# langtech-bsc/quantool

Measured on AMD Instinct MI355X. Metric: quantized weights/sec (GPTQ int4, Llama-3-8B, 512 calib samples), higher is better.
Workload: dtype f32

## Files before the change

quantool_amd/csrc/build.py:

```python
from __future__ import annotations

import hashlib
import os
import shutil
import subprocess
import sys
from concurrent.futures import ThreadPoolExecutor
from pathlib import Path

CSRC = Path(__file__).resolve().parent
PKG = CSRC.parent
LIB_DIR = PKG / "lib"
OBJ_DIR = CSRC / "_obj"
LIB_PATH = LIB_DIR / "libquantool_hip.so"

HIPCC_FLAGS = [
    "--offload-arch=gfx950",
    "-O3",
    "-fPIC",
    "-std=c++17",
    "-ffp-contract=off",
    "-fhip-fp32-correctly-rounded-divide-sqrt",
    "-fno-fast-math",
    "-Wall",
# ... 55 lines not shown
        if m:
            kv = m.group(1).strip()
            if kv.startswith("Function Name:"):
                cur = {"name": kv.split(":", 1)[1].strip()}
                kernels.append(cur)
            elif cur is not None and ":" in kv:
                k, v = kv.rsplit(":", 1)
                cur[k.strip()] = v.strip()
            while i + 1 < len(lines) and re.match(r"^\s+\d* ?\|", lines[i + 1]):
                i += 1
        elif not re.match(r"^\d+ (warning|remark)s? generated", line.strip()) and "remarks generated" not in line:
            rest.append(line)
        i += 1
    rows = []
    for k in kernels:
        rows.append(f"{k['name']}\tvgpr {k.get('VGPRs', '?')}\tagpr {k.get('AGPRs', '?')}\tscratch "
                    f"{k.get('ScratchSize [bytes/lane]', '?')}\tvgpr_spill {k.get('VGPRs Spill', '?')}\tlds "
                    f"{k.get('LDS Size [bytes/block]', '?')}\twaves_per_simd {k.get('Occupancy [waves/SIMD]', '?')}")
    (OBJ_DIR / (src.stem + ".resources.txt")).write_text("\n".join(rows) + ("\n" if rows else ""))
    bad = [k["name"] for k in kernels
           if k.get("ScratchSize [bytes/lane]", "0") not in ("0", "?") and not any(ok in k["name"] for ok in SCRATCH_OK)]
    if bad:
        raise RuntimeError(f"{src.name}: kernel(s) with a private segment (scratch): {bad} -- see "
                           f"{OBJ_DIR / (src.stem + '.resources.txt')}; a by-value argument struct that is modified and "
                           "indexed at run time, or a register array indexed at run time, is the usual cause")
    return "\n".join(rest) + ("\n" if rest else "")


def audit_m0(src: Path) -> None:
    stamp = OBJ_DIR / (src.stem + ".m0audit")
    want = _stamp(src)
    if stamp.exists() and stamp.read_text() == want:
        return
    asm = OBJ_DIR / (src.stem + ".device.s")
    cmd = [_hipcc(), *[f for f in HIPCC_FLAGS if f != "-fPIC"], "--cuda-device-only", "-S", str(src), "-o", str(asm)]
    res = subprocess.run(cmd, capture_output=True, text=True)
    if res.returncode != 0:
        raise RuntimeError(f"hipcc -S failed for {src.name}:\n{res.stderr}")
    inside = False
    for n, line in enumerate(asm.read_text().splitlines(), 1):
        if ";;#ASMSTART" in line:
            inside = True
        elif ";;#ASMEND" in line:
            inside = False
        elif not inside and "m0" in line.split(";")[0].replace("_m0", ""):
            raise RuntimeError(f"{src.name}: compiler-generated use of M0 at {asm.name}:{n}: {line.strip()!r} -- "
                               "the LDS-DMA helpers must save/restore M0 again")
    audit_spills(src.name, asm.read_text())
    asm.unlink()
    stamp.write_text(want)


NO_SPILL_KERNELS = ("xtx_kernel", "xtx16_kernel", "gemm3_kernel", "sgemm_ring_kernel", "quantize_tokens_kernel",
                    "gemm_i8_kernel")


def audit_spills(src_name: str, asm_text: str) -> None:
    name = None
    for line in asm_text.splitlines():
        t = line.strip()
        if t.startswith(".name:"):
            name = t.split(":", 1)[1].strip()
        elif name and t.startswith((".vgpr_spill_count:", ".private_segment_fixed_size:")):
            if int(t.split(":", 1)[1]) != 0 and any(k in name for k in NO_SPILL_KERNELS):
                raise RuntimeError(f"{src_name}: {name} spills ({t}) -- its schedule assumes every value stays in registers")


def build(verbose: bool = False) -> Path:
    OBJ_DIR.mkdir(exist_ok=True)
    LIB_DIR.mkdir(exist_ok=True)
    srcs = sources()
    with ThreadPoolExecutor(max_workers=min(8, len(srcs))) as ex:
        objs = list(ex.map(_compile, srcs))
    for name in ("xtx.hip", "gemm3_tn.hip", "sgemm_tn.hip", "qlinear.hip"):
        audit_m0(CSRC / name)
    newest = max(o.stat().st_mtime for o in objs)
    if not LIB_PATH.exists() or LIB_PATH.stat().st_mtime < newest:
        cmd = [_hipcc(), "--offload-arch=gfx950", "-shared", "-fPIC", "-o", str(LIB_PATH), *map(str, objs)]
        res = subprocess.run(cmd, capture_output=True, text=True)
        if res.returncode != 0:
            raise RuntimeError(f"link failed:\n{res.stdout}\n{res.stderr}")
    if verbose:
        print(f"built {LIB_PATH}")
    return LIB_PATH


if __name__ == "__main__":
    build(verbose=True)
```

quantool_amd/csrc/cholesky.hip:

```cpp
#include <stdlib.h>
#include <string.h>

#include <map>
#include <tuple>
#include <vector>

#include "common.h"
#include "gemm3_tn.h"
#include "sgemm_tn.h"

namespace {

constexpr int NB = 128;
constexpr int NBO_MAX = 1024;
static int chol_block_env(const char* name) {
    const char* e = getenv(name);
    if (!e) return 0;
    int x = atoi(e) / 128 * 128;
    return x < 128 ? 128 : (x > NBO_MAX ? NBO_MAX : x);
}
struct G3Step {
    int n_items = 0, n_red = 0;
    size_t item_off = 0, red_off = 0;
};
// ... 47 lines not shown
        for (const G3Red& r : red) pl->max_slabs = pl->max_slabs > r.first + r.count ? pl->max_slabs : r.first + r.count;
        pl->any = true;
        return st;
    };
    for (int J0 = 0; J0 < K; J0 += NBO) {
        const int J1 = (K - J0 < NBO) ? K : J0 + NBO;
        pl->fac.push_back(J0 == 0 ? G3Step() : add((J1 - J0 + 255) / 256, (K - J0 + 255) / 256, J0 / G3_CHUNK_ROWS, 0));
    }
    for (int I0 = 0; I0 < K; I0 += NBI) {
        const int I1 = (K - I0 < NBI) ? K : I0 + NBI;
        pl->inv.push_back(I0 == 0 ? G3Step() : add((I1 - I0 + 255) / 256, (I0 + 255) / 256, I0 / G3_CHUNK_ROWS, 1));
    }
    if (pl->any) {
        pl->blob_bytes = qt_align_up(bytes.size(), 256);
        if (hipHostMalloc((void**)&pl->blob, pl->blob_bytes, hipHostMallocDefault) != hipSuccess) {
            pl->any = false;
            pl->blob = nullptr;
        } else {
            memcpy(pl->blob, bytes.data(), bytes.size());
        }
    }
    if (!pl->any) {
        pl->blob_bytes = 0;
        pl->max_slabs = 0;
        for (G3Step& st : pl->fac) st = G3Step();
        for (G3Step& st : pl->inv) st = G3Step();
    }
    plans[key] = pl;
    return pl;
}
static size_t chol_g3_ws_bytes(const CholG3Plan* pl, int K) {
    if (!pl->any) return 0;
    return 2 * qt_align_up((size_t)3 * K * K * 2, 256) + (size_t)pl->max_slabs * 256 * 256 * 4 + pl->blob_bytes + 256;
}

static const CholG3Plan* chol_blocks(int K, int& NBO, int& NBI) {
    const int eo = chol_block_env("QT_CHOL_NBO"), ei = chol_block_env("QT_CHOL_NBI");
    NBO = eo ? eo : 512;
    NBI = ei ? ei : 512;
    const CholG3Plan* pl = chol_g3_plan(K, NBO, NBI);
    if (pl->any) return pl;
    NBO = eo ? eo : 256;
    NBI = ei ? ei : 256;
    return chol_g3_plan(K, NBO, NBI);
}

constexpr int LDP = NB + 1;

constexpr int LDT = NB + 4;
constexpr int RD_STRIDE = NB * NB + 4 * 32 * 32;

#define QT_SEL4(kb, v0, v1, v2, v3) ((kb) == 0 ? (v0) : (kb) == 1 ? (v1) : (kb) == 2 ? (v2) : (v3))

constexpr int LDA = NB + 4;

__device__ __forceinline__ float readlane_f(float v, int lane) {
    return __int_as_float(__builtin_amdgcn_readlane(__float_as_int(v), lane));
}

__device__ __forceinline__ void mma32_tn(const float* A, int lda, const float* B, int ldb, f32x16& acc,
                                         int l31, int h, bool negate_a) {
#pragma unroll
    for (int kk = 0; kk < 16; ++kk) {
        float a = A[(2 * kk + h) * lda + l31];
        const float b = B[(2 * kk + h) * ldb + l31];
        if (negate_a) a = -a;
        acc = __builtin_amdgcn_mfma_f32_32x32x2f32(a, b, acc, 0, 0, 0);
    }
}

constexpr int POTF2_THREADS = 512, POTF2_WAVES = POTF2_THREADS / 64;
__global__ __launch_bounds__(POTF2_THREADS) void potf2_kernel(const float* P, int64_t ldp, int n,
                                                    float* Rout, int64_t ldr,
                                                    float* __restrict__ Rd, int32_t* info, int col0, int prio,
                                                    int64_t bsP, int64_t bsRd) {
    qt_set_chain_prio(prio);
    if (blockIdx.x) {
        P += (size_t)blockIdx.x * bsP;
        Rout += (size_t)blockIdx.x * bsP;
        Rd += (size_t)blockIdx.x * bsRd;
        info += blockIdx.x;
    }
    extern __shared__ __attribute__((aligned(16))) float sm[];
    float* As = sm;
    float* Xs = sm + NB * LDA;
    const int tid = threadIdx.x, lane = tid & 63;
    const int wave = __builtin_amdgcn_readfirstlane(tid >> 6);
    const int l31 = lane & 31, h = lane >> 5;

    if ((ldp & 3) == 0 && (n & 3) == 0 && (((uintptr_t)P) & 15) == 0) {
        constexpr int NV = NB * NB / 4 / POTF2_THREADS;
        f32x4 v[NV];
#pragma unroll
        for (int r = 0; r < NV; ++r) {
            const int e4 = tid + POTF2_THREADS * r;
            const int i = e4 >> 5, j = (e4 & 31) * 4;
            const int ic = i < n ? i : n - 1, jc = j < n ? j : n - 4;
            v[r] = *(const f32x4*)(P + (size_t)ic * ldp + jc);
        }
#pragma unroll
        for (int r = 0; r < NV; ++r) {
            const int e4 = tid + POTF2_THREADS * r;
            const int i = e4 >> 5, j = (e4 & 31) * 4;
            f32x4 x;
#pragma unroll
            for (int q = 0; q < 4; ++q) x[q] = (i < n && j + q < n) ? v[r][q] : (i == j + q ? 1.0f : 0.0f);
            *(f32x4*)(As + i * LDA + j) = x;
        }
    } else {
        for (int e = tid; e < NB * NB; e += POTF2_THREADS) {
            const int i = e / NB, j = e % NB;
            const int lo = i < j ? i : j, hi = i < j ? j : i;
            float v = (i == j) ? 1.0f : 0.0f;
            if (hi < n) v = P[(size_t)lo * ldp + hi];
            As[i * LDA + j] = v;
        }
    }
    __syncthreads();

    int bad = 0;
#pragma unroll 1
    for (int kb = 0; kb < 4; ++kb) {
        float* Akk = As + (32 * kb) * LDA + 32 * kb;
        if (wave == 0) {
            f32x16 c1, c2;
#pragma unroll
            for (int r = 0; r < 16; ++r) {
                const int i = (r & 3) + 8 * (r >> 2) + 4 * h;
                c1[r] = Akk[i * LDA + l31];
                c2[r] = (i == l31) ? 1.0f : 0.0f;
            }
#pragma unroll
            for (int c = 0; c < 32; ++c) {
                const int rc = (c & 3) + 4 * (c >> 3);
                const int hc = (c >> 2) & 1;
                float piv = readlane_f(c1[rc], c + 32 * hc);
                const bool isbad = !(piv > 0.0f);
                bad = (isbad && bad == 0 && 32 * kb + c < n) ? 32 * kb + c + 1 : bad;
                piv = isbad ? 1.0f : piv;
                float rs = __builtin_amdgcn_rsqf(piv);
                rs = rs * fmaf(-0.5f * piv * rs, rs, 1.5f);
                const bool mine = h == hc;
                const float rr = c1[rc] * rs, zz = c2[rc] * rs;
                c1[rc] = mine ? rr : c1[rc];
                c2[rc] = mine ? zz : c2[rc];
                if (c < 31) {
                    const float a = (mine && l31 > c) ? -rr : 0.0f;
                    const float b1 = (mine && l31 >= c) ? rr : 0.0f, b2 = mine ? zz : 0.0f;
                    c1 = __builtin_amdgcn_mfma_f32_32x32x2f32(a, b1, c1, 0, 0, 0);
                    c2 = __builtin_amdgcn_mfma_f32_32x32x2f32(a, b2, c2, 0, 0, 0);
                }
            }
#pragma unroll
            for (int r = 0; r < 16; ++r) {
                const int i = (r & 3) + 8 * (r >> 2) + 4 * h;
                Akk[i * LDA + l31] = (i <= l31) ? c1[r] : 0.0f;
                Xs[(kb * 32 + l31) * 32 + i] = (i >= l31) ? c2[r] : 0.0f;
            }
        }
        __syncthreads();
        if (kb == 3) break;
        for (int a = kb + 1 + wave; a < 4; a += POTF2_WAVES) {
            f32x16 acc;
#pragma unroll
            for (int r = 0; r < 16; ++r) acc[r] = 0.0f;
            float* Bt = As + (32 * kb) * LDA + 32 * a;
            mma32_tn(Xs + kb * 1024, 32, Bt, LDA, acc, l31, h, false);
#pragma unroll
            for (int r = 0; r < 16; ++r) Bt[((r & 3) + 8 * (r >> 2) + 4 * h) * LDA + l31] = acc[r];
        }
        __syncthreads();
        {
            int t = 0;
            for (int a = kb + 1; a < 4; ++a)
                for (int a2 = a; a2 < 4; ++a2, ++t) {
                    if ((t % POTF2_WAVES) != wave) continue;
                    float* Ct = As + (32 * a) * LDA + 32 * a2;
                    f32x16 acc;
#pragma unroll
                    for (int r = 0; r < 16; ++r) acc[r] = Ct[((r & 3) + 8 * (r >> 2) + 4 * h) * LDA + l31];
                    mma32_tn(As + (32 * kb) * LDA + 32 * a, LDA, As + (32 * kb) * LDA + 32 * a2, LDA, acc, l31, h,
                             true);
#pragma unroll
                    for (int r = 0; r < 16; ++r) Ct[((r & 3) + 8 * (r >> 2) + 4 * h) * LDA + l31] = acc[r];
                }
        }
        __syncthreads();
    }
    if (bad != 0 && tid == 0) atomicCAS(info, 0, col0 + bad);
    const bool vec_out = (ldr & 3) == 0 && (n & 3) == 0 && (((uintptr_t)Rout) & 15) == 0;
    for (int e4 = tid; e4 < NB * NB / 4; e4 += POTF2_THREADS) {
        const int i = e4 >> 5, j = (e4 & 31) * 4;
        f32x4 v = *(const f32x4*)(As + i * LDA + j);
#pragma unroll
        for (int q = 0; q < 4; ++q) v[q] = (j + q >= i) ? v[q] : 0.0f;
        *(f32x4*)(Rd + i * NB + j) = v;
        if (i < n && j + 3 >= i && j < n) {
            if (vec_out) {
                *(f32x4*)(Rout + (size_t)i * ldr + j) = v;
            } else {
#pragma unroll
                for (int q = 0; q < 4; ++q)
                    if (j + q >= i && j + q < n) Rout[(size_t)i * ldr + j + q] = v[q];
            }
        }
    }
    for (int e4 = tid; e4 < 4 * 32 * 32 / 4; e4 += POTF2_THREADS) *(f32x4*)(Rd + NB * NB + 4 * e4) = *(const f32x4*)(Xs + 4 * e4);
}

__global__ __launch_bounds__(256) void trsm_rt_kernel(const float* __restrict__ Rd, int n,
                                                      const float* B, int64_t ldb,
                                                      float* Z, int64_t ldz, int ncols, int prio, int64_t bsRd,
                                                      int64_t bsB) {
    qt_set_chain_prio(prio);
    if (blockIdx.y) {
        Rd += (size_t)blockIdx.y * bsRd;
        B += (size_t)blockIdx.y * bsB;
        Z += (size_t)blockIdx.y * bsB;
    }
    extern __shared__ __attribute__((aligned(16))) float Rs[];
    const int tid = threadIdx.x, lane = tid & 63, wave = tid >> 6;
    const float* D32 = Rs + NB * NB;
    const int l31 = lane & 31, h = lane >> 5;
    const int col = blockIdx.x * 128 + wave * 32 + l31;
    const bool cok = col < ncols;
    const int colc = cok ? col : ncols - 1;

    f32x16 acc[4];
#pragma unroll
    for (int a = 0; a < 4; ++a)
#pragma unroll
        for (int r = 0; r < 16; ++r) {
            const int row = 32 * a + (r & 3) + 8 * (r >> 2) + 4 * h;
            acc[a][r] = (row < n) ? B[(size_t)row * ldb + colc] : 0.0f;
        }
    {
        constexpr int NV = RD_STRIDE / 4 / 256;
        static_assert(NV * 4 * 256 == RD_STRIDE, "whole float4s per thread");
        f32x4 v[NV];
#pragma unroll
        for (int r = 0; r < NV; ++r) v[r] = ((const f32x4*)Rd)[tid + 256 * r];
#pragma unroll
        for (int r = 0; r < NV; ++r) ((f32x4*)Rs)[tid + 256 * r] = v[r];
    }
    __syncthreads();

#pragma unroll
    for (int b = 0; b < 4; ++b) {
        f32x16 zb;
#pragma unroll
        for (int r = 0; r < 16; ++r) zb[r] = 0.0f;
#pragma unroll
        for (int r = 0; r < 16; ++r) {
            const int k = (r & 3) + 8 * (r >> 2) + 4 * h;
            const float av = D32[(b * 32 + k) * 32 + l31];
            zb = __builtin_amdgcn_mfma_f32_32x32x2f32(av, acc[b][r], zb, 0, 0, 0);
        }
        acc[b] = zb;
#pragma unroll
        for (int a = b + 1; a < 4; ++a) {
#pragma unroll
            for (int r = 0; r < 16; ++r) {
                const int k = (r & 3) + 8 * (r >> 2) + 4 * h;
                const float av = -Rs[(32 * b + k) * NB + 32 * a + l31];
                acc[a] = __builtin_amdgcn_mfma_f32_32x32x2f32(av, zb[r], acc[a], 0, 0, 0);
            }
        }
    }
    if (cok) {
#pragma unroll
        for (int a = 0; a < 4; ++a)
#pragma unroll
            for (int r = 0; r < 16; ++r) {
                const int row = 32 * a + (r & 3) + 8 * (r >> 2) + 4 * h;
                if (row < n) Z[(size_t)row * ldz + col] = acc[a][r];
            }
    }
}

__global__ __launch_bounds__(128) void trinv_batched_kernel(const float* __restrict__ Rd_all, int K,
                                                            float* __restrict__ Dinv_all,
                                                            float* __restrict__ Y, int64_t ldy, int64_t bsW, int64_t bsY) {
    if (blockIdx.y) {
        Rd_all += (size_t)blockIdx.y * bsW;
        Dinv_all += (size_t)blockIdx.y * bsW;
        Y += (size_t)blockIdx.y * bsY;
    }
    extern __shared__ __attribute__((aligned(16))) float sm[];
    float* Rt = sm;
    float* Xs = sm + NB * LDT;
    const int b = blockIdx.x;
    const int n = (K - b * NB < NB) ? K - b * NB : NB;
    const float* Rd = Rd_all + (size_t)b * RD_STRIDE;
    const int j = threadIdx.x;
    for (int e = j; e < NB * NB; e += NB) {
        const int i = e / NB, c = e % NB;
        Rt[c * LDT + i] = Rd[e];
    }
    __syncthreads();
    float x0[32], x1[32], x2[32], x3[32];
#pragma unroll
    for (int r = 0; r < 32; ++r) {
        x0[r] = (r == j) ? 1.0f : 0.0f;
        x1[r] = (32 + r == j) ? 1.0f : 0.0f;
        x2[r] = (64 + r == j) ? 1.0f : 0.0f;
        x3[r] = (96 + r == j) ? 1.0f : 0.0f;
    }
#pragma unroll 1
    for (int pb = 3; pb >= 0; --pb) {
#pragma unroll
        for (int pp = 31; pp >= 0; --pp) {
            const int p = 32 * pb + pp;
            const float* rp = Rt + p * LDT;
            const float xp = QT_SEL4(pb, x0[pp], x1[pp], x2[pp], x3[pp]) / rp[p];
            if (pb == 0) x0[pp] = xp;
            if (pb == 1) x1[pp] = xp;
            if (pb == 2) x2[pp] = xp;
            if (pb == 3) x3[pp] = xp;
#define QT_XUPD(arr, a, r_to)                                                 \
    _Pragma("unroll") for (int r4 = 0; r4 < (r_to); r4 += 4) {                 \
        const f32x4 v4 = *(const f32x4*)(rp + 32 * (a) + r4);                 \
        _Pragma("unroll") for (int e = 0; e < 4; ++e)                         \
            if (r4 + e < (r_to)) arr[r4 + e] = fmaf(-v4[e], xp, arr[r4 + e]); \
    }
            if (pb == 0) { QT_XUPD(x0, 0, pp) } else { QT_XUPD(x0, 0, 32) }
            if (pb == 1) { QT_XUPD(x1, 1, pp) } else if (pb > 1) { QT_XUPD(x1, 1, 32) }
            if (pb == 2) { QT_XUPD(x2, 2, pp) } else if (pb > 2) { QT_XUPD(x2, 2, 32) }
            if (pb == 3) { QT_XUPD(x3, 3, pp) }
#undef QT_XUPD
        }
// ... 179 lines not shown
    const size_t split_ws_bytes = (size_t)2048 * NB * NB * 4 + (size_t)NBO_MAX * K * 4;
    unsigned short *Rpl = nullptr, *Ypl = nullptr;
    float* g3_slabs = nullptr;
    char* g3_tab = nullptr;
    const int64_t plane_stride = (int64_t)K * K;
    if (g3->any) {
        char* q = (char*)qt_align_up((size_t)((char*)split_ws + split_ws_bytes), 256);
        Rpl = (unsigned short*)q;
        q += qt_align_up((size_t)3 * K * K * 2, 256);
        Ypl = (unsigned short*)q;
        q += qt_align_up((size_t)3 * K * K * 2, 256);
        g3_slabs = (float*)q;
        g3_tab = (char*)qt_align_up((size_t)(ws + (size_t)nprob * prob_bytes), 256);
        QT_HIP(hipMemcpyAsync(g3_tab, g3->blob, g3->blob_bytes, hipMemcpyHostToDevice, stream));
    }
    auto g3_row = [&](const G3Step& st, const unsigned short* Bplanes, int col_a0, int col_b0, int M, int N, float* C,
                      int64_t bsC, int mode) -> int {
        G3Args a;
        a.Apl = Rpl;
        a.Bpl = Bplanes;
        a.plane_stride = plane_stride;
        a.ld = K;
        a.rowA0 = a.rowB0 = 0;
        a.colA0 = col_a0;
        a.colB0 = col_b0;
        a.colmax = K;
        a.M = M;
        a.N = N;
        a.C = C;
        a.ldc = K;
        a.mode = mode;
        a.slabs = g3_slabs;
        a.items = (const G3Item*)(g3_tab + st.item_off);
        a.n_items = st.n_items;
        a.red = (const G3Red*)(g3_tab + st.red_off);
        a.n_red = st.n_red;
        a.batch = nprob;
        a.bsApl = a.bsBpl = sW * 2;
        a.bsC = bsC;
        a.bsSlabs = sW;
        return qt_gemm3_launch(a, stream);
    };
    auto sgemm = [&](SgemmArgs& g, int64_t bsA_, int64_t bsB_, int64_t bsC_) -> int {
        g.batch = nprob;
        g.bsA = bsA_;
        g.bsB = bsB_;
        g.bsCin = g.bsCout = bsC_;
        g.bs_split = sW;
        return qt_sgemm_tn(g, stream);
    };
    float* Y = U;
    const int64_t sY = sU;
    const size_t inv_lds = (size_t)(NB * LDT + NB * LDP) * sizeof(float);
    const size_t potf2_lds = (size_t)(NB * LDA + 4 * 32 * 32) * sizeof(float);
    static QtOncePerDevice lds_attr;
    QT_HIP(lds_attr.run([&] {
        hipError_t e = hipFuncSetAttribute((const void*)potf2_kernel, hipFuncAttributeMaxDynamicSharedMemorySize,
                                           (int)potf2_lds);
        if (e == hipSuccess)
            e = hipFuncSetAttribute((const void*)trsm_rt_kernel, hipFuncAttributeMaxDynamicSharedMemorySize,
                                    (int)(RD_STRIDE * sizeof(float)));
        if (e == hipSuccess)
            e = hipFuncSetAttribute((const void*)trinv_batched_kernel, hipFuncAttributeMaxDynamicSharedMemorySize,
                                    (int)inv_lds);
        if (e == hipSuccess)
            e = hipFuncSetAttribute((const void*)trinv_mfma_kernel, hipFuncAttributeMaxDynamicSharedMemorySize,
                                    (int)(RD_STRIDE * sizeof(float)));
        return e;
    }));
    QT_HIP(hipMemsetAsync(info, 0, sizeof(int32_t) * nprob, stream));
    const int prio = qt_chain_prio();

    for (int J0 = 0, Jb = 0; J0 < K; J0 += NBO, ++Jb) {
        const int J1 = (K - J0 < NBO) ? K : J0 + NBO;
        if (g3->any && J0 > 0) {
            const G3Step& st = g3->fac[Jb];
            float* C = A + (size_t)J0 * K + J0;
            if (st.n_items > 0) {
                int rc = g3_row(st, Rpl, J0, J0, J1 - J0, K - J0, C, sA, G3_SUB);
                if (rc) return rc;
            } else {
                SgemmArgs g;
                g.A = A + J0; g.lda = K;
                g.B = A + J0; g.ldb = K;
                g.Cin = C; g.ldcin = K;
                g.Cout = C; g.ldcout = K;
                g.M = J1 - J0; g.N = K - J0; g.kdim = J0; g.k_mode = SG_K_FULL; g.mode = SG_MODE_SUB;
                g.split_ws = split_ws; g.split_ws_bytes = split_ws_bytes;
                int rc = sgemm(g, sA, sA, sA);
                if (rc) return rc;
            }
        }
        for (int j0 = J0; j0 < J1; j0 += NB) {
            const int j = j0 / NB, nbj = (K - j0 < NB) ? K - j0 : NB;
            float* Ajj = A + (size_t)j0 * K + j0;
            if (j0 > J0) {
                SgemmArgs g;
                g.A = A + (size_t)J0 * K + j0; g.lda = K;
                g.B = A + (size_t)J0 * K + j0; g.ldb = K;
                g.Cin = Ajj; g.ldcin = K;
                g.Cout = Ajj; g.ldcout = K;
                g.M = nbj; g.N = K - j0; g.kdim = j0 - J0; g.k_mode = SG_K_FULL; g.mode = SG_MODE_SUB;
                int rc = sgemm(g, sA, sA, sA);
                if (rc) return rc;
            }
            hipLaunchKernelGGL(potf2_kernel, dim3(nprob), dim3(POTF2_THREADS), potf2_lds, stream, (const float*)Ajj, (int64_t)K, nbj,
                               Ajj, (int64_t)K, Rd + (size_t)j * RD_STRIDE, info, j0, prio, sA, sW);
            QT_LAUNCH_CHECK();
            const int rest = K - j0 - nbj;
            if (rest > 0) {
                hipLaunchKernelGGL(trsm_rt_kernel, dim3((rest + 127) / 128, nprob), dim3(256), RD_STRIDE * sizeof(float),
                                   stream, (const float*)(Rd + (size_t)j * RD_STRIDE), nbj, (const float*)(Ajj + nbj),
                                   (int64_t)K, Ajj + nbj, (int64_t)K, rest, prio, sW, sA);
                QT_LAUNCH_CHECK();
            }
        }
        const int rem = K - J1;
        if (g3->any) {
            if (rem > 0) {
                int rc = qt_split3_launch(A + (size_t)J0 * K + J0, K, J1 - J0, K - J0, Rpl + (size_t)J0 * K + J0, K,
                                          plane_stride, 0, 0, 0, stream, nprob, sA, sW * 2);
                if (rc) return rc;
            }
        } else if (rem > 0) {
            SgemmArgs g;
            g.A = A + (size_t)J0 * K + J1; g.lda = K;
            g.B = A + (size_t)J0 * K + J1; g.ldb = K;
            g.Cin = A + (size_t)J1 * K + J1; g.ldcin = K;
            g.Cout = A + (size_t)J1 * K + J1; g.ldcout = K;
            g.M = rem; g.N = rem; g.kdim = J1 - J0; g.k_mode = SG_K_FULL; g.mode = SG_MODE_SUB;
            g.upper_only = 1;
            int rc = sgemm(g, sA, sA, sA);
            if (rc) return rc;
        }
    }
    {
        const char* e = getenv("QT_CHOL_TRINV");
        if (e && strcmp(e, "div") == 0)
            hipLaunchKernelGGL(trinv_batched_kernel, dim3(nblk, nprob), dim3(NB), inv_lds, stream, (const float*)Rd, K, Dinv, Y,
                               (int64_t)K, sW, sY);
        else
            hipLaunchKernelGGL(trinv_mfma_kernel, dim3(nblk, nprob), dim3(256), RD_STRIDE * sizeof(float), stream,
                               (const float*)Rd, K, Dinv, Y, (int64_t)K, sW, sY);
    }
    QT_LAUNCH_CHECK();
    for (int I0 = 0, Ib = 0; I0 < K; I0 += NBI, ++Ib) {
        const int I1 = (K - I0 < NBI) ? K : I0 + NBI;
        const int Wi = I1 - I0;
        for (int i0 = I0 + NB; i0 < I1; i0 += NB) {
            const int i = i0 / NB, nbi = (K - i0 < NB) ? K - i0 : NB;
            SgemmArgs g;
            g.A = A + (size_t)I0 * K + i0; g.lda = K;
            g.B = Y + (size_t)I0 * K + I0; g.ldb = K;
            g.Cin = nullptr; g.ldcin = 0;
            g.Cout = T; g.ldcout = K;
            g.M = nbi; g.N = i0 - I0; g.kdim = i0 - I0; g.k_mode = SG_K_FROM_N0; g.mode = SG_MODE_SET;
            int rc = sgemm(g, sA, sY, sW);
            if (rc) return rc;
            SgemmArgs t;
            t.A = Dinv + (size_t)i * NB * NB; t.lda = NB;
            t.B = T; t.ldb = K;
            t.Cin = nullptr; t.ldcin = 0;
            t.Cout = Y + (size_t)i0 * K + I0; t.ldcout = K;
            t.M = nbi; t.N = i0 - I0; t.kdim = nbi; t.k_mode = SG_K_FULL; t.mode = SG_MODE_NEG;
            rc = sgemm(t, sW, sW, sY);
            if (rc) return rc;
// ... 63 lines not shown
```

Before: 2.564 billion.

## Register-resident panel Cholesky and streamed-operand TRSM to cut LDS and raise occupancy

The 128x128 diagonal-block Cholesky kernel changes from 512 threads holding the whole block in LDS to 256 threads, where each wave keeps up to three 32x32 tiles in MFMA accumulator registers. Only a single 32-row strip and a 32x33 inverse tile stay in shared memory, and each output strip is written out as it finishes. The TRSM kernel no longer stages the 64KB+ Rd block in LDS. It reads operands directly with buffer loads through a 12-deep register prefetch ring, unrolled at compile time. Both kernels drop their dynamic LDS, ask for 5 waves per EU, and are added to the spill and M0 audits. The intent is higher occupancy and less LDS traffic on the Cholesky critical path, at the cost of register pressure and a harder-to-maintain compile-time schedule.

```diff
diff --git a/quantool_amd/csrc/build.py b/quantool_amd/csrc/build.py
--- a/quantool_amd/csrc/build.py
+++ b/quantool_amd/csrc/build.py
@@ -131,7 +131,7 @@
 
 
 NO_SPILL_KERNELS = ("xtx_kernel", "xtx16_kernel", "gemm3_kernel", "sgemm_ring_kernel", "quantize_tokens_kernel",
-                    "gemm_i8_kernel")
+                    "gemm_i8_kernel", "potf2_kernel", "trsm_rt_kernel")
 
 
 def audit_spills(src_name: str, asm_text: str) -> None:
@@ -151,7 +151,7 @@
     srcs = sources()
     with ThreadPoolExecutor(max_workers=min(8, len(srcs))) as ex:
         objs = list(ex.map(_compile, srcs))
-    for name in ("xtx.hip", "gemm3_tn.hip", "sgemm_tn.hip", "qlinear.hip"):
+    for name in ("xtx.hip", "gemm3_tn.hip", "sgemm_tn.hip", "qlinear.hip", "cholesky.hip"):
         audit_m0(CSRC / name)
     newest = max(o.stat().st_mtime for o in objs)
     if not LIB_PATH.exists() or LIB_PATH.stat().st_mtime < newest:
diff --git a/quantool_amd/csrc/cholesky.hip b/quantool_amd/csrc/cholesky.hip
--- a/quantool_amd/csrc/cholesky.hip
+++ b/quantool_amd/csrc/cholesky.hip
@@ -123,7 +123,8 @@
 
 #define QT_SEL4(kb, v0, v1, v2, v3) ((kb) == 0 ? (v0) : (kb) == 1 ? (v1) : (kb) == 2 ? (v2) : (v3))
 
-constexpr int LDA = NB + 4;
+constexpr int LDS_S = NB + 4;
+constexpr int LDX = 33;
 
 __device__ __forceinline__ float readlane_f(float v, int lane) {
     return __int_as_float(__builtin_amdgcn_readlane(__float_as_int(v), lane));
@@ -140,67 +141,64 @@
     }
 }
 
-constexpr int POTF2_THREADS = 512, POTF2_WAVES = POTF2_THREADS / 64;
-__global__ __launch_bounds__(POTF2_THREADS) void potf2_kernel(const float* P, int64_t ldp, int n,
-                                                    float* Rout, int64_t ldr,
-                                                    float* __restrict__ Rd, int32_t* info, int col0, int prio,
-                                                    int64_t bsP, int64_t bsRd) {
-    qt_set_chain_prio(prio);
-    if (blockIdx.x) {
-        P += (size_t)blockIdx.x * bsP;
-        Rout += (size_t)blockIdx.x * bsP;
-        Rd += (size_t)blockIdx.x * bsRd;
-        info += blockIdx.x;
-    }
-    extern __shared__ __attribute__((aligned(16))) float sm[];
-    float* As = sm;
-    float* Xs = sm + NB * LDA;
-    const int tid = threadIdx.x, lane = tid & 63;
-    const int wave = __builtin_amdgcn_readfirstlane(tid >> 6);
+__device__ __forceinline__ void strip_store(float* S, int cb, const f32x16& t, int l31, int h) {
+#pragma unroll
+    for (int r = 0; r < 16; ++r) S[((r & 3) + 8 * (r >> 2) + 4 * h) * LDS_S + 32 * cb + l31] = t[r];
+}
+
+template <int W, int S_>
+struct Potf2Tile {
+    static constexpr int a = S_ == 0 ? W : S_ == 1 ? (0x37B6 >> (4 * W) & 15) >> 2 : ((W == 1 || W == 2) ? 0 : -1);
+    static constexpr int b = S_ == 0 ? W : S_ == 1 ? (0x37B6 >> (4 * W) & 15) & 3 : ((W == 1 || W == 2) ? W : -1);
+};
+
+constexpr int POTF2_THREADS = 256, POTF2_SLOTS = 3;
+
+template <int W>
+__device__ __forceinline__ void potf2_wave(const float* P, int64_t ldp, int n, float* Rout, int64_t ldr, float* Rd,
+                                           float* S, float* Xs, int* bad_s, int tid, int lane) {
+    constexpr int ta[POTF2_SLOTS] = {Potf2Tile<W, 0>::a, Potf2Tile<W, 1>::a, Potf2Tile<W, 2>::a};
+    constexpr int tb[POTF2_SLOTS] = {Potf2Tile<W, 0>::b, Potf2Tile<W, 1>::b, Potf2Tile<W, 2>::b};
     const int l31 = lane & 31, h = lane >> 5;
 
-    if ((ldp & 3) == 0 && (n & 3) == 0 && (((uintptr_t)P) & 15) == 0) {
-        constexpr int NV = NB * NB / 4 / POTF2_THREADS;
-        f32x4 v[NV];
-#pragma unroll
-        for (int r = 0; r < NV; ++r) {
-            const int e4 = tid + POTF2_THREADS * r;
-            const int i = e4 >> 5, j = (e4 & 31) * 4;
-            const int ic = i < n ? i : n - 1, jc = j < n ? j : n - 4;
-            v[r] = *(const f32x4*)(P + (size_t)ic * ldp + jc);
-        }
-#pragma unroll
-        for (int r = 0; r < NV; ++r) {
-            const int e4 = tid + POTF2_THREADS * r;
-            const int i = e4 >> 5, j = (e4 & 31) * 4;
-            f32x4 x;
-#pragma unroll
-            for (int q = 0; q < 4; ++q) x[q] = (i < n && j + q < n) ? v[r][q] : (i == j + q ? 1.0f : 0.0f);
-            *(f32x4*)(As + i * LDA + j) = x;
-        }
-    } else {
-        for (int e = tid; e < NB * NB; e += POTF2_THREADS) {
-            const int i = e / NB, j = e % NB;
+    f32x16 t[POTF2_SLOTS];
+#pragma unroll
+    for (int s = 0; s < POTF2_SLOTS; ++s) {
+        if (ta[s] < 0) continue;
+#pragma unroll
+        for (int r = 0; r < 16; ++r) {
+            const int i = 32 * ta[s] + (r & 3) + 8 * (r >> 2) + 4 * h, j = 32 * tb[s] + l31;
             const int lo = i < j ? i : j, hi = i < j ? j : i;
-            float v = (i == j) ? 1.0f : 0.0f;
-            if (hi < n) v = P[(size_t)lo * ldp + hi];
-            As[i * LDA + j] = v;
-        }
-    }
-    __syncthreads();
-
-    int bad = 0;
-#pragma unroll 1
+            t[s][r] = P[(size_t)(lo < n ? lo : n - 1) * ldp + (hi < n ? hi : n - 1)];
+        }
+        __builtin_amdgcn_sched_barrier(0);
+    }
+    asm volatile("s_waitcnt vmcnt(0)" ::: "memory");
+    const int dl = l31 - 4 * h;
+#pragma unroll
+    for (int s = 0; s < POTF2_SLOTS; ++s) {
+        if (ta[s] < 0) continue;
+        const int off = dl + 32 * (tb[s] - ta[s]);
+        const bool jin = l31 < n - 32 * tb[s];
+#pragma unroll
+        for (int r = 0; r < 16; ++r) {
+            const int rho = (r & 3) + 8 * (r >> 2);
+            t[s][r] = (rho <= off) ? (jin ? t[s][r] : (rho == off ? 1.0f : 0.0f)) : 0.0f;
+        }
+    }
+
+    const bool vec_out = (ldr & 3) == 0 && (n & 3) == 0 && (((uintptr_t)Rout) & 15) == 0;
+#pragma unroll
     for (int kb = 0; kb < 4; ++kb) {
-        float* Akk = As + (32 * kb) * LDA + 32 * kb;
-        if (wave == 0) {
-            f32x16 c1, c2;
-#pragma unroll
-            for (int r = 0; r < 16; ++r) {
-                const int i = (r & 3) + 8 * (r >> 2) + 4 * h;
-                c1[r] = Akk[i * LDA + l31];
-                c2[r] = (i == l31) ? 1.0f : 0.0f;
-            }
+#pragma unroll
+        for (int s = 1; s < POTF2_SLOTS; ++s)
+            if (ta[s] == kb) strip_store(S, tb[s], t[s], l31, h);
+        if (W == kb) {
+            f32x16& c1 = t[0];
+            f32x16 c2;
+            int bad = 0;
+#pragma unroll
+            for (int r = 0; r < 16; ++r) c2[r] = ((r & 3) + 8 * (r >> 2) + 4 * h == l31) ? 1.0f : 0.0f;
 #pragma unroll
             for (int c = 0; c < 32; ++c) {
                 const int rc = (c & 3) + 4 * (c >> 3);
@@ -221,132 +219,198 @@
                     c1 = __builtin_amdgcn_mfma_f32_32x32x2f32(a, b1, c1, 0, 0, 0);
                     c2 = __builtin_amdgcn_mfma_f32_32x32x2f32(a, b2, c2, 0, 0, 0);
                 }
+                __builtin_amdgcn_sched_barrier(0);
             }
 #pragma unroll
             for (int r = 0; r < 16; ++r) {
                 const int i = (r & 3) + 8 * (r >> 2) + 4 * h;
-                Akk[i * LDA + l31] = (i <= l31) ? c1[r] : 0.0f;
-                Xs[(kb * 32 + l31) * 32 + i] = (i >= l31) ? c2[r] : 0.0f;
+                S[i * LDS_S + 32 * kb + l31] = (i <= l31) ? c1[r] : 0.0f;
+                Xs[l31 * LDX + i] = (i >= l31) ? c2[r] : 0.0f;
             }
+            if (lane == 0) bad_s[kb] = bad;
         }
         __syncthreads();
-        if (kb == 3) break;
-        for (int a = kb + 1 + wave; a < 4; a += POTF2_WAVES) {
-            f32x16 acc;
-#pragma unroll
-            for (int r = 0; r < 16; ++r) acc[r] = 0.0f;
-            float* Bt = As + (32 * kb) * LDA + 32 * a;
-            mma32_tn(Xs + kb * 1024, 32, Bt, LDA, acc, l31, h, false);
-#pragma unroll
-            for (int r = 0; r < 16; ++r) Bt[((r & 3) + 8 * (r >> 2) + 4 * h) * LDA + l31] = acc[r];
-        }
-        __syncthreads();
-        {
-            int t = 0;
-            for (int a = kb + 1; a < 4; ++a)
-                for (int a2 = a; a2 < 4; ++a2, ++t) {
-                    if ((t % POTF2_WAVES) != wave) continue;
-                    float* Ct = As + (32 * a) * LDA + 32 * a2;
-                    f32x16 acc;
-#pragma unroll
-                    for (int r = 0; r < 16; ++r) acc[r] = Ct[((r & 3) + 8 * (r >> 2) + 4 * h) * LDA + l31];
-                    mma32_tn(As + (32 * kb) * LDA + 32 * a, LDA, As + (32 * kb) * LDA + 32 * a2, LDA, acc, l31, h,
-                             true);
-#pragma unroll
-                    for (int r = 0; r < 16; ++r) Ct[((r & 3) + 8 * (r >> 2) + 4 * h) * LDA + l31] = acc[r];
+        if (kb < 3) {
+#pragma unroll
+            for (int s = 1; s < POTF2_SLOTS; ++s)
+                if (ta[s] == kb) {
+#pragma unroll
+                    for (int r = 0; r < 16; ++r) t[s][r] = 0.0f;
+                    mma32_tn(Xs, LDX, S + 32 * tb[s], LDS_S, t[s], l31, h, false);
+                    strip_store(S, tb[s], t[s], l31, h);
+                    __builtin_amdgcn_sched_barrier(0);
                 }
-        }
-        __syncthreads();
-    }
-    if (bad != 0 && tid == 0) atomicCAS(info, 0, col0 + bad);
-    const bool vec_out = (ldr & 3) == 0 && (n & 3) == 0 && (((uintptr_t)Rout) & 15) == 0;
-    for (int e4 = tid; e4 < NB * NB / 4; e4 += POTF2_THREADS) {
-        const int i = e4 >> 5, j = (e4 & 31) * 4;
-        f32x4 v = *(const f32x4*)(As + i * LDA + j);
-#pragma unroll
-        for (int q = 0; q < 4; ++q) v[q] = (j + q >= i) ? v[q] : 0.0f;
-        *(f32x4*)(Rd + i * NB + j) = v;
-        if (i < n && j + 3 >= i && j < n) {
-            if (vec_out) {
-                *(f32x4*)(Rout + (size_t)i * ldr + j) = v;
-            } else {
-#pragma unroll
-                for (int q = 0; q < 4; ++q)
-                    if (j + q >= i && j + q < n) Rout[(size_t)i * ldr + j + q] = v[q];
+            __syncthreads();
+#pragma unroll
+            for (int s = 0; s < POTF2_SLOTS; ++s)
+                if (ta[s] > kb) {
+                    mma32_tn(S + 32 * ta[s], LDS_S, S + 32 * tb[s], LDS_S, t[s], l31, h, true);
+                    __builtin_amdgcn_sched_barrier(0);
+                }
+        }
+        const int k0 = tid >> 5, j = (tid & 31) * 4, orow = k0 * (int)ldr + j;
+#pragma unroll
+        for (int q4 = 0; q4 < 32 * 32 / POTF2_THREADS; ++q4) {
+            const int k = k0 + 8 * q4, i = 32 * kb + k;
+            float* Rrow = Rout + (size_t)(32 * kb + 8 * q4) * ldr;
+            f32x4 v = *(const f32x4*)(S + k * LDS_S + j);
+#pragma unroll
+            for (int q = 0; q < 4; ++q) v[q] = (j + q >= i) ? v[q] : 0.0f;
+            *(f32x4*)(Rd + (32 * kb + 8 * q4) * NB + (k0 * NB + j)) = v;
+            if (i < n && j + 3 >= i && j < n) {
+                if (vec_out) {
+                    *(f32x4*)(Rrow + orow) = v;
+                } else {
+#pragma unroll
+                    for (int q = 0; q < 4; ++q)
+                        if (j + q >= i && j + q < n) Rrow[orow + q] = v[q];
+                }
             }
         }
-    }
-    for (int e4 = tid; e4 < 4 * 32 * 32 / 4; e4 += POTF2_THREADS) *(f32x4*)(Rd + NB * NB + 4 * e4) = *(const f32x4*)(Xs + 4 * e4);
-}
-
-__global__ __launch_bounds__(256) void trsm_rt_kernel(const float* __restrict__ Rd, int n,
-                                                      const float* B, int64_t ldb,
-                                                      float* Z, int64_t ldz, int ncols, int prio, int64_t bsRd,
-                                                      int64_t bsB) {
+#pragma unroll
+        for (int q = 0; q < 32 * 32 / POTF2_THREADS; ++q) {
+            const int e = tid + POTF2_THREADS * q;
+            Rd[NB * NB + kb * 1024 + e] = Xs[(e >> 5) * LDX + (e & 31)];
+        }
+        if (kb < 3) __syncthreads();
+    }
+}
+
+__global__ __launch_bounds__(POTF2_THREADS) __attribute__((amdgpu_waves_per_eu(5))) void potf2_kernel(
+        const float* P, int64_t ldp, int n, float* Rout, int64_t ldr, float* __restrict__ Rd, int32_t* info, int col0,
+        int prio, int64_t bsP, int64_t bsRd) {
+    qt_set_chain_prio(prio);
+    if (blockIdx.x) {
+        P += (size_t)blockIdx.x * bsP;
+        Rout += (size_t)blockIdx.x * bsP;
+        Rd += (size_t)blockIdx.x * bsRd;
+        info += blockIdx.x;
+    }
+    __shared__ __attribute__((aligned(16))) float S[32 * LDS_S];
+    __shared__ float Xs[32 * LDX];
+    __shared__ int bad_s[4];
+    const int tid = threadIdx.x, lane = tid & 63;
+    switch (__builtin_amdgcn_readfirstlane(tid >> 6)) {
+        case 0: potf2_wave<0>(P, ldp, n, Rout, ldr, Rd, S, Xs, bad_s, tid, lane); break;
+        case 1: potf2_wave<1>(P, ldp, n, Rout, ldr, Rd, S, Xs, bad_s, tid, lane); break;
+        case 2: potf2_wave<2>(P, ldp, n, Rout, ldr, Rd, S, Xs, bad_s, tid, lane); break;
+        default: potf2_wave<3>(P, ldp, n, Rout, ldr, Rd, S, Xs, bad_s, tid, lane); break;
+    }
+    if (tid == 0) {
+        int bad = 0;
+        for (int b = 0; b < 4 && bad == 0; ++b) bad = bad_s[b];
+        if (bad != 0) atomicCAS(info, 0, col0 + bad);
+    }
+}
+
+struct TrsmStep {
+    int b, a, r;
+};
+__device__ constexpr TrsmStep trsm_step(int g) {
+    const int G = g / 16, b = G < 4 ? 0 : G < 7 ? 1 : G < 9 ? 2 : 3, first = b == 0 ? 0 : b == 1 ? 4 : b == 2 ? 7 : 9;
+    return TrsmStep{b, b + G - first, g % 16};
+}
+__device__ constexpr int trsm_soff(int g) {
+    const TrsmStep st = trsm_step(g);
+    const int rho = (st.r & 3) + 8 * (st.r >> 2);
+    return st.a == st.b ? (NB * NB + (32 * st.b + rho) * 32) * 4 : ((32 * st.b + rho) * NB + 32 * st.a) * 4;
+}
+constexpr int TRSM_STEPS = 160, TRSM_PD = 12;
+
+struct TrsmCtx {
+    f32x16 acc[4], zb;
+    float ring[TRSM_PD];
+    __amdgpu_buffer_rsrc_t rs;
+    int vR, vD, n, col, colc, h;
+    bool cok;
+    const float* B;
+    int64_t ldb;
+    float* Z;
+    int64_t ldz;
+};
+
+__device__ __forceinline__ float trsm_operand(const TrsmCtx& c, int g) {
+    return __builtin_bit_cast(float, __builtin_amdgcn_raw_buffer_load_b32(
+                                         c.rs, trsm_step(g).a == trsm_step(g).b ? c.vD : c.vR, trsm_soff(g), 0));
+}
+
+__device__ __forceinline__ void trsm_load_rows(TrsmCtx& c, int a) {
+    if (c.n == NB) {
+#pragma unroll
+        for (int r = 0; r < 16; ++r) {
+            const int row = 32 * a + (r & 3) + 8 * (r >> 2) + 4 * c.h;
+            c.acc[a][r] = c.B[(size_t)row * c.ldb + c.colc];
+        }
+    } else {
+#pragma unroll
+        for (int r = 0; r < 16; ++r) {
+            const int row = 32 * a + (r & 3) + 8 * (r >> 2) + 4 * c.h;
+            c.acc[a][r] = (row < c.n) ? c.B[(size_t)row * c.ldb + c.colc] : 0.0f;
+        }
+    }
+}
+
+template <int g>
+__device__ __forceinline__ void trsm_steps(TrsmCtx& c) {
+    if constexpr (g < TRSM_STEPS) {
+        constexpr TrsmStep st = trsm_step(g);
+        const float av = c.ring[g % TRSM_PD];
+        if constexpr (g + TRSM_PD < TRSM_STEPS) c.ring[g % TRSM_PD] = trsm_operand(c, g + TRSM_PD);
+        if constexpr (st.a == st.b) {
+            if constexpr (st.r == 0)
+#pragma unroll
+                for (int r = 0; r < 16; ++r) c.zb[r] = 0.0f;
+            c.zb = __builtin_amdgcn_mfma_f32_32x32x2f32(av, c.acc[st.b][st.r], c.zb, 0, 0, 0);
+            if constexpr (st.r == 15) {
+                if (c.cok) {
+#pragma unroll
+                    for (int r = 0; r < 16; ++r) {
+                        const int row = 32 * st.b + (r & 3) + 8 * (r >> 2) + 4 * c.h;
+                        if (row < c.n) c.Z[(size_t)row * c.ldz + c.col] = c.zb[r];
+                    }
+                }
+            }
+        } else {
+            c.acc[st.a] = __builtin_amdgcn_mfma_f32_32x32x2f32(-av, c.zb[st.r], c.acc[st.a], 0, 0, 0);
+        }
+        if constexpr (g == 15) {
+            trsm_load_rows(c, 2);
+            trsm_load_rows(c, 3);
+        }
+        __builtin_amdgcn_sched_barrier(0);
+        trsm_steps<g + 1>(c);
+    }
+}
+
+__global__ __launch_bounds__(256) __attribute__((amdgpu_waves_per_eu(5))) void trsm_rt_kernel(
+        const float* __restrict__ Rd, int n, const float* B, int64_t ldb, float* Z, int64_t ldz, int ncols, int prio,
+        int64_t bsRd, int64_t bsB) {
     qt_set_chain_prio(prio);
     if (blockIdx.y) {
         Rd += (size_t)blockIdx.y * bsRd;
         B += (size_t)blockIdx.y * bsB;
         Z += (size_t)blockIdx.y * bsB;
     }
-    extern __shared__ __attribute__((aligned(16))) float Rs[];
     const int tid = threadIdx.x, lane = tid & 63, wave = tid >> 6;
-    const float* D32 = Rs + NB * NB;
     const int l31 = lane & 31, h = lane >> 5;
-    const int col = blockIdx.x * 128 + wave * 32 + l31;
-    const bool cok = col < ncols;
-    const int colc = cok ? col : ncols - 1;
-
-    f32x16 acc[4];
-#pragma unroll
-    for (int a = 0; a < 4; ++a)
-#pragma unroll
-        for (int r = 0; r < 16; ++r) {
-            const int row = 32 * a + (r & 3) + 8 * (r >> 2) + 4 * h;
-            acc[a][r] = (row < n) ? B[(size_t)row * ldb + colc] : 0.0f;
-        }
-    {
-        constexpr int NV = RD_STRIDE / 4 / 256;
-        static_assert(NV * 4 * 256 == RD_STRIDE, "whole float4s per thread");
-        f32x4 v[NV];
-#pragma unroll
-        for (int r = 0; r < NV; ++r) v[r] = ((const f32x4*)Rd)[tid + 256 * r];
-#pragma unroll
-        for (int r = 0; r < NV; ++r) ((f32x4*)Rs)[tid + 256 * r] = v[r];
-    }
-    __syncthreads();
-
-#pragma unroll
-    for (int b = 0; b < 4; ++b) {
-        f32x16 zb;
-#pragma unroll
-        for (int r = 0; r < 16; ++r) zb[r] = 0.0f;
-#pragma unroll
-        for (int r = 0; r < 16; ++r) {
-            const int k = (r & 3) + 8 * (r >> 2) + 4 * h;
-            const float av = D32[(b * 32 + k) * 32 + l31];
-            zb = __builtin_amdgcn_mfma_f32_32x32x2f32(av, acc[b][r], zb, 0, 0, 0);
-        }
-        acc[b] = zb;
-#pragma unroll
-        for (int a = b + 1; a < 4; ++a) {
-#pragma unroll
-            for (int r = 0; r < 16; ++r) {
-                const int k = (r & 3) + 8 * (r >> 2) + 4 * h;
-                const float av = -Rs[(32 * b + k) * NB + 32 * a + l31];
-                acc[a] = __builtin_amdgcn_mfma_f32_32x32x2f32(av, zb[r], acc[a], 0, 0, 0);
-            }
-        }
-    }
-    if (cok) {
-#pragma unroll
-        for (int a = 0; a < 4; ++a)
-#pragma unroll
-            for (int r = 0; r < 16; ++r) {
-                const int row = 32 * a + (r & 3) + 8 * (r >> 2) + 4 * h;
-                if (row < n) Z[(size_t)row * ldz + col] = acc[a][r];
-            }
-    }
+    TrsmCtx c;
+    c.col = blockIdx.x * 128 + wave * 32 + l31;
+    c.cok = c.col < ncols;
+    c.colc = c.cok ? c.col : ncols - 1;
+    c.rs = __builtin_amdgcn_make_buffer_rsrc((void*)Rd, 0, RD_STRIDE * 4, 0x00020000);
+    c.vR = (4 * h * NB + l31) * 4;
+    c.vD = (4 * h * 32 + l31) * 4;
+    c.n = n;
+    c.h = h;
+    c.B = B;
+    c.ldb = ldb;
+    c.Z = Z;
+    c.ldz = ldz;
+    trsm_load_rows(c, 0);
+    trsm_load_rows(c, 1);
+#pragma unroll
+    for (int g = 0; g < TRSM_PD; ++g) c.ring[g] = trsm_operand(c, g);
+    trsm_steps<0>(c);
 }
 
 __global__ __launch_bounds__(128) void trinv_batched_kernel(const float* __restrict__ Rd_all, int K,
@@ -632,16 +696,9 @@
     float* Y = U;
     const int64_t sY = sU;
     const size_t inv_lds = (size_t)(NB * LDT + NB * LDP) * sizeof(float);
-    const size_t potf2_lds = (size_t)(NB * LDA + 4 * 32 * 32) * sizeof(float);
     static QtOncePerDevice lds_attr;
     QT_HIP(lds_attr.run([&] {
-        hipError_t e = hipFuncSetAttribute((const void*)potf2_kernel, hipFuncAttributeMaxDynamicSharedMemorySize,
-                                           (int)potf2_lds);
-        if (e == hipSuccess)
-            e = hipFuncSetAttribute((const void*)trsm_rt_kernel, hipFuncAttributeMaxDynamicSharedMemorySize,
-                                    (int)(RD_STRIDE * sizeof(float)));
-        if (e == hipSuccess)
-            e = hipFuncSetAttribute((const void*)trinv_batched_kernel, hipFuncAttributeMaxDynamicSharedMemorySize,
+        hipError_t e = hipFuncSetAttribute((const void*)trinv_batched_kernel, hipFuncAttributeMaxDynamicSharedMemorySize,
                                     (int)inv_lds);
         if (e == hipSuccess)
             e = hipFuncSetAttribute((const void*)trinv_mfma_kernel, hipFuncAttributeMaxDynamicSharedMemorySize,
@@ -684,13 +741,12 @@
                 int rc = sgemm(g, sA, sA, sA);
                 if (rc) return rc;
             }
-            hipLaunchKernelGGL(potf2_kernel, dim3(nprob), dim3(POTF2_THREADS), potf2_lds, stream, (const float*)Ajj, (int64_t)K, nbj,
+            hipLaunchKernelGGL(potf2_kernel, dim3(nprob), dim3(POTF2_THREADS), 0, stream, (const float*)Ajj, (int64_t)K, nbj,
                                Ajj, (int64_t)K, Rd + (size_t)j * RD_STRIDE, info, j0, prio, sA, sW);
             QT_LAUNCH_CHECK();
             const int rest = K - j0 - nbj;
             if (rest > 0) {
-                hipLaunchKernelGGL(trsm_rt_kernel, dim3((rest + 127) / 128, nprob), dim3(256), RD_STRIDE * sizeof(float),
-                                   stream, (const float*)(Rd + (size_t)j * RD_STRIDE), nbj, (const float*)(Ajj + nbj),
+                hipLaunchKernelGGL(trsm_rt_kernel, dim3((rest + 127) / 128, nprob), dim3(256), 0, stream, (const float*)(Rd + (size_t)j * RD_STRIDE), nbj, (const float*)(Ajj + nbj),
                                    (int64_t)K, Ajj + nbj, (int64_t)K, rest, prio, sW, sA);
                 QT_LAUNCH_CHECK();
             }
```

Result: no change. 2.579 billion (median of 6 runs) (+0.6%).

## Add register-tiled MFMA panel Cholesky and trsm kernels as default path

Applied to the files above, without the earlier changes.

Adds a new panel factorization kernel that holds the 128x128 diagonal block as 32x32 tiles in MFMA accumulator registers, spread over four waves. It factors each diagonal 32x32 tile with an MFMA-based rank-1 loop and also builds that tile's inverse. It also adds a trsm kernel that applies these inverse diagonal tiles across 32-column strips, using a small LDS exchange between waves. The new path becomes the default, and the old kernels are kept behind QT_CHOL_PANEL=r4. The aim is to cut the LDS traffic and latency of the panel step on the critical path, at the cost of smaller trsm blocks and possible precision or occupancy changes.

```diff
diff --git a/quantool_amd/csrc/cholesky.hip b/quantool_amd/csrc/cholesky.hip
--- a/quantool_amd/csrc/cholesky.hip
+++ b/quantool_amd/csrc/cholesky.hip
@@ -346,6 +346,220 @@
                 const int row = 32 * a + (r & 3) + 8 * (r >> 2) + 4 * h;
                 if (row < n) Z[(size_t)row * ldz + col] = acc[a][r];
             }
+    }
+}
+
+constexpr int CR_THREADS = 256;
+constexpr int CR_LDP = NB + 4;
+
+__device__ __forceinline__ int cr_tile(int wave, int s) {
+    const int t1 = wave == 0 ? 1 : wave == 1 ? 2 : wave == 2 ? 3 : 7;
+    const int t2 = wave == 1 ? 11 : wave == 2 ? 6 : -1;
+    return s == 0 ? 5 * wave : s == 1 ? t1 : t2;
+}
+
+__device__ __forceinline__ int potf2_diag32(f32x16& c1, f32x16& c2, int kb, int n, int l31, int h) {
+    int bad = 0;
+#pragma unroll
+    for (int r = 0; r < 16; ++r) {
+        const int i = (r & 3) + 8 * (r >> 2) + 4 * h;
+        c2[r] = (i == l31) ? 1.0f : 0.0f;
+    }
+#pragma unroll
+    for (int c = 0; c < 32; ++c) {
+        int lim = n - 32 * kb;
+        asm volatile("" : "+v"(l31), "+s"(lim));
+        const int rc = (c & 3) + 4 * (c >> 3);
+        const int hc = (c >> 2) & 1;
+        float piv = readlane_f(c1[rc], c + 32 * hc);
+        const bool isbad = !(piv > 0.0f);
+        bad = (isbad && bad == 0 && c < lim) ? 32 * kb + c + 1 : bad;
+        piv = isbad ? 1.0f : piv;
+        float rs = __builtin_amdgcn_rsqf(piv);
+        rs = rs * fmaf(-0.5f * piv * rs, rs, 1.5f);
+        const bool mine = h == hc;
+        const float rr = c1[rc] * rs, zz = c2[rc] * rs;
+        c1[rc] = mine ? rr : c1[rc];
+        c2[rc] = mine ? zz : c2[rc];
+        if (c < 31) {
+            const float a = (mine && l31 > c) ? -rr : 0.0f;
+            const float b1 = (mine && l31 >= c) ? rr : 0.0f, b2 = mine ? zz : 0.0f;
+            c1 = __builtin_amdgcn_mfma_f32_32x32x2f32(a, b1, c1, 0, 0, 0);
+            c2 = __builtin_amdgcn_mfma_f32_32x32x2f32(a, b2, c2, 0, 0, 0);
+        }
+    }
+    return bad;
+}
+
+template <bool DIAG>
+__device__ __forceinline__ void potf2_cr_slot(int phase, int tc, f32x16& t, int kb, int n, int lane, float* Pn, float* Xs,
+                                              int* bad_s) {
+    const int l31 = lane & 31, h = lane >> 5;
+    if (tc < 0) return;
+    const int a = tc >> 2, a2 = tc & 3;
+    if (phase == 0 && a == kb) {
+        float* Tp = Pn + 32 * a2;
+        if (DIAG) {
+            f32x16 c2;
+            const int bad = potf2_diag32(t, c2, kb, n, l31, h);
+            if (bad != 0 && lane == 0 && *bad_s == 0) *bad_s = bad;
+#pragma unroll
+            for (int r = 0; r < 16; ++r) {
+                const int i = (r & 3) + 8 * (r >> 2) + 4 * h;
+                Tp[i * CR_LDP + l31] = (i <= l31) ? t[r] : 0.0f;
+                Xs[l31 * 32 + i] = (i >= l31) ? c2[r] : 0.0f;
+            }
+        } else {
+#pragma unroll
+            for (int r = 0; r < 16; ++r) Tp[((r & 3) + 8 * (r >> 2) + 4 * h) * CR_LDP + l31] = t[r];
+        }
+    } else if (!DIAG && phase == 1 && a == kb) {
+        float* Bt = Pn + 32 * a2;
+        f32x16 acc;
+#pragma unroll
+        for (int r = 0; r < 16; ++r) acc[r] = 0.0f;
+        mma32_tn(Xs, 32, Bt, CR_LDP, acc, l31, h, false);
+#pragma unroll
+        for (int r = 0; r < 16; ++r) Bt[((r & 3) + 8 * (r >> 2) + 4 * h) * CR_LDP + l31] = acc[r];
+    } else if (phase == 2 && a > kb) {
+        mma32_tn(Pn + 32 * a, CR_LDP, Pn + 32 * a2, CR_LDP, t, l31, h, true);
+    }
+}
+
+__global__ __launch_bounds__(CR_THREADS) __attribute__((amdgpu_waves_per_eu(5)))
+void potf2_cr_kernel(const float* P, int64_t ldp, int n, float* Rout, int64_t ldr, float* __restrict__ Rd, int32_t* info,
+                     int col0, int prio, int64_t bsP, int64_t bsRd) {
+    qt_set_chain_prio(prio);
+    if (blockIdx.x) {
+        P += (size_t)blockIdx.x * bsP;
+        Rout += (size_t)blockIdx.x * bsP;
+        Rd += (size_t)blockIdx.x * bsRd;
+        info += blockIdx.x;
+    }
+    __shared__ __attribute__((aligned(16))) float Pn[32 * CR_LDP];
+    __shared__ __attribute__((aligned(16))) float Xs[32 * 32];
+    __shared__ int bad_s;
+    const int tid = threadIdx.x, lane = tid & 63;
+    const int wave = __builtin_amdgcn_readfirstlane(tid >> 6);
+    const int h = lane >> 5, l31 = lane & 31;
+    if (tid == 0) bad_s = 0;
+    const int tc0 = cr_tile(wave, 0), tc1 = cr_tile(wave, 1), tc2 = cr_tile(wave, 2);
+
+    const int ldp32 = (int)ldp;
+    auto load = [&](int tc, f32x16& t) {
+        const int a = tc < 0 ? 0 : tc >> 2, a2 = tc & 3;
+        const int j = 32 * a2 + l31, jc = j < n ? j : n - 1;
+#pragma unroll
+        for (int r = 0; r < 16; ++r) {
+            const int i = 32 * a + (r & 3) + 8 * (r >> 2) + 4 * h, ic = i < n ? i : n - 1;
+            const float v = P[ic * ldp32 + jc];
+            t[r] = (tc >= 0 && i < n && j < n && i <= j) ? v : ((i == j) ? 1.0f : 0.0f);
+        }
+    };
+    f32x16 t0, t1, t2;
+    load(tc0, t0);
+    load(tc1, t1);
+    load(tc2, t2);
+    const bool vec_out = (ldr & 3) == 0 && (n & 3) == 0 && (((uintptr_t)Rout) & 15) == 0;
+#pragma unroll 1
+    for (int kb = 0; kb < 4; ++kb) {
+        int lk = lane, tk = tid;
+        asm volatile("" : "+v"(lk), "+v"(tk));
+        potf2_cr_slot<true>(0, tc0, t0, kb, n, lk, Pn, Xs, &bad_s);
+        potf2_cr_slot<false>(0, tc1, t1, kb, n, lk, Pn, Xs, &bad_s);
+        potf2_cr_slot<false>(0, tc2, t2, kb, n, lk, Pn, Xs, &bad_s);
+        __syncthreads();
+        if (kb < 3) {
+            potf2_cr_slot<true>(1, tc0, t0, kb, n, lk, Pn, Xs, &bad_s);
+            potf2_cr_slot<false>(1, tc1, t1, kb, n, lk, Pn, Xs, &bad_s);
+            potf2_cr_slot<false>(1, tc2, t2, kb, n, lk, Pn, Xs, &bad_s);
+            __syncthreads();
+            potf2_cr_slot<true>(2, tc0, t0, kb, n, lk, Pn, Xs, &bad_s);
+            potf2_cr_slot<false>(2, tc1, t1, kb, n, lk, Pn, Xs, &bad_s);
+            potf2_cr_slot<false>(2, tc2, t2, kb, n, lk, Pn, Xs, &bad_s);
+        }
+        for (int e4 = tk; e4 < 32 * NB / 4; e4 += CR_THREADS) {
+            const int i = 32 * kb + (e4 >> 5), j = (e4 & 31) * 4;
+            f32x4 v = *(const f32x4*)(Pn + (e4 >> 5) * CR_LDP + j);
+#pragma unroll
+            for (int q = 0; q < 4; ++q) v[q] = (j + q >= i) ? v[q] : 0.0f;
+            *(f32x4*)(Rd + i * NB + j) = v;
+            if (i < n && j + 3 >= i && j < n) {
+                if (vec_out) {
+                    *(f32x4*)(Rout + (size_t)i * ldr + j) = v;
+                } else {
+#pragma unroll
+                    for (int q = 0; q < 4; ++q)
+                        if (j + q >= i && j + q < n) Rout[(size_t)i * ldr + j + q] = v[q];
+                }
+            }
+        }
+        *(f32x4*)(Rd + NB * NB + kb * 1024 + 4 * tk) = *(const f32x4*)(Xs + 4 * tk);
+        __syncthreads();
+    }
+    if (tid == 0 && bad_s != 0) atomicCAS(info, 0, col0 + bad_s);
+}
+
+__global__ __launch_bounds__(CR_THREADS) __attribute__((amdgpu_waves_per_eu(5)))
+void trsm_cr_kernel(const float* __restrict__ Rd, int n, const float* B, int64_t ldb, float* Z, int64_t ldz, int ncols,
+                    int prio, int64_t bsRd, int64_t bsB) {
+    qt_set_chain_prio(prio);
+    if (blockIdx.y) {
+        Rd += (size_t)blockIdx.y * bsRd;
+        B += (size_t)blockIdx.y * bsB;
+        Z += (size_t)blockIdx.y * bsB;
+    }
+    __shared__ __attribute__((aligned(16))) float Zs[3 * 16 * 64];
+    const int tid = threadIdx.x, lane = tid & 63;
+    const int a = __builtin_amdgcn_readfirstlane(tid >> 6);
+    const int l31 = lane & 31, h = lane >> 5;
+    const int col = blockIdx.x * 32 + l31;
+    const bool cok = col < ncols;
+    const int colc = cok ? col : ncols - 1;
+
+    f32x16 acc, xa;
+#pragma unroll
+    for (int r = 0; r < 16; ++r) {
+        const int k = (r & 3) + 8 * (r >> 2) + 4 * h;
+        const int row = 32 * a + k;
+        acc[r] = (row < n) ? B[(size_t)row * ldb + colc] : 0.0f;
+        xa[r] = Rd[NB * NB + (a * 32 + k) * 32 + l31];
+    }
+#pragma unroll
+    for (int b = 0; b < 4; ++b) {
+        if (a == b) {
+            f32x16 zb;
+#pragma unroll
+            for (int r = 0; r < 16; ++r) zb[r] = 0.0f;
+#pragma unroll
+            for (int r = 0; r < 16; ++r) zb = __builtin_amdgcn_mfma_f32_32x32x2f32(xa[r], acc[r], zb, 0, 0, 0);
+            acc = zb;
+            if (b < 3) {
+#pragma unroll
+                for (int r = 0; r < 16; ++r) Zs[(b * 16 + r) * 64 + lane] = zb[r];
+            }
+        }
+        if (b == 3) break;
+        f32x16 rv;
+        if (a > b) {
+#pragma unroll
+            for (int r = 0; r < 16; ++r) {
+                const int k = (r & 3) + 8 * (r >> 2) + 4 * h;
+                rv[r] = -Rd[(32 * b + k) * NB + 32 * a + l31];
+            }
+        }
+        __syncthreads();
+        if (a > b) {
+#pragma unroll
+            for (int r = 0; r < 16; ++r) acc = __builtin_amdgcn_mfma_f32_32x32x2f32(rv[r], Zs[(b * 16 + r) * 64 + lane], acc, 0, 0, 0);
+        }
+    }
+    if (cok) {
+#pragma unroll
+        for (int r = 0; r < 16; ++r) {
+            const int row = 32 * a + (r & 3) + 8 * (r >> 2) + 4 * h;
+            if (row < n) Z[(size_t)row * ldz + col] = acc[r];
+        }
     }
 }
 
@@ -650,6 +864,8 @@
     }));
     QT_HIP(hipMemsetAsync(info, 0, sizeof(int32_t) * nprob, stream));
     const int prio = qt_chain_prio();
+    const char* panel_env = getenv("QT_CHOL_PANEL");
+    const bool panel_r4 = panel_env && strcmp(panel_env, "r4") == 0;
 
     for (int J0 = 0, Jb = 0; J0 < K; J0 += NBO, ++Jb) {
         const int J1 = (K - J0 < NBO) ? K : J0 + NBO;
@@ -684,14 +900,23 @@
                 int rc = sgemm(g, sA, sA, sA);
                 if (rc) return rc;
             }
-            hipLaunchKernelGGL(potf2_kernel, dim3(nprob), dim3(POTF2_THREADS), potf2_lds, stream, (const float*)Ajj, (int64_t)K, nbj,
-                               Ajj, (int64_t)K, Rd + (size_t)j * RD_STRIDE, info, j0, prio, sA, sW);
+            if (panel_r4)
+                hipLaunchKernelGGL(potf2_kernel, dim3(nprob), dim3(POTF2_THREADS), potf2_lds, stream, (const float*)Ajj, (int64_t)K,
+                                   nbj, Ajj, (int64_t)K, Rd + (size_t)j * RD_STRIDE, info, j0, prio, sA, sW);
+            else
+                hipLaunchKernelGGL(potf2_cr_kernel, dim3(nprob), dim3(CR_THREADS), 0, stream, (const float*)Ajj, (int64_t)K, nbj,
+                                   Ajj, (int64_t)K, Rd + (size_t)j * RD_STRIDE, info, j0, prio, sA, sW);
             QT_LAUNCH_CHECK();
             const int rest = K - j0 - nbj;
             if (rest > 0) {
-                hipLaunchKernelGGL(trsm_rt_kernel, dim3((rest + 127) / 128, nprob), dim3(256), RD_STRIDE * sizeof(float),
-                                   stream, (const float*)(Rd + (size_t)j * RD_STRIDE), nbj, (const float*)(Ajj + nbj),
-                                   (int64_t)K, Ajj + nbj, (int64_t)K, rest, prio, sW, sA);
+                if (panel_r4)
+                    hipLaunchKernelGGL(trsm_rt_kernel, dim3((rest + 127) / 128, nprob), dim3(256), RD_STRIDE * sizeof(float),
+                                       stream, (const float*)(Rd + (size_t)j * RD_STRIDE), nbj, (const float*)(Ajj + nbj),
+                                       (int64_t)K, Ajj + nbj, (int64_t)K, rest, prio, sW, sA);
+                else
+                    hipLaunchKernelGGL(trsm_cr_kernel, dim3((rest + 31) / 32, nprob), dim3(CR_THREADS), 0, stream,
+                                       (const float*)(Rd + (size_t)j * RD_STRIDE), nbj, (const float*)(Ajj + nbj), (int64_t)K,
+                                       Ajj + nbj, (int64_t)K, rest, prio, sW, sA);
                 QT_LAUNCH_CHECK();
             }
         }
```

Measured after the change: 2.993 billion before, 3.008 billion after (median of 6 runs). About the same (+0.5%).
